# unixpickle/learn-nerf

Measured on AMD Instinct MI355X. Metric: ray-samples/s (NeRF train step: fwd + bwd + Adam, 4096 rays x 192 samples per GPU), higher is better.
Workload: dtype bf16; 1 GPU; vanilla NeRF coarse64+fine128 train step (BASELINE.json configs[1]); rays_per_gpu=4096, coarse_samples=64, fine_samples=128, global_batch_rays=4096, parallelism=dp1, precision=bf16 MFMA, fp32 accumulate/master weights

## Files before the change

learn-nerf_amd/csrc/fused_chain.h:

```cpp
#pragma once
#include <utility>

#include "common.h"
#include "fast_math.h"
#include "nerf_wgrad.h"

namespace lnrf {
using namespace nl;

typedef __bf16 bf16x8 __attribute__((ext_vector_type(8)));
typedef float f32x16 __attribute__((ext_vector_type(16)));
typedef float f32x4 __attribute__((ext_vector_type(4)));
typedef short s16x4 __attribute__((ext_vector_type(4)));


template <class F, int... I>
__device__ __forceinline__ void static_for_impl(F&& f, std::integer_sequence<int, I...>) {
  (f(std::integral_constant<int, I>{}), ...);
}
template <int N, class F>
__device__ __forceinline__ void static_for(F&& f) {
  static_for_impl(f, std::make_integer_sequence<int, N>{});
}

constexpr int kThreads = kWaves * 64;
constexpr int kStageBytes = kStageFrags * kFragBytes;
constexpr int kSlots = 3;
constexpr int kRingBytes = kSlots * kStageBytes;
constexpr int kBiasLdsOff = kRingBytes;
constexpr int kFragAhead = 4;

extern __shared__ __attribute__((aligned(16))) char smem[];

#ifdef LNRF_TIMELINE
struct Timeline {
  unsigned long long* buf = nullptr;
  int n = 0;
  bool on = false;
  __device__ __forceinline__ void stamp() {
    if (on) {
      const unsigned long long t = __builtin_amdgcn_s_memtime();
      if ((threadIdx.x & 63) == 0) buf[(threadIdx.x >> 6) * 1024 + n] = t;
      ++n;
    }
  }
};
#define LNRF_TL_STAMP(ring) (ring).tl.stamp()
#else
#define LNRF_TL_STAMP(ring) ((void)0)
#endif

__device__ __forceinline__ bf16x8 bits_to_frag(uint4 v) { return __builtin_bit_cast(bf16x8, v); }
__device__ __forceinline__ uint4 frag_to_bits(bf16x8 v) { return __builtin_bit_cast(uint4, v); }
__device__ __forceinline__ bf16x8 zero_frag() { return bits_to_frag(make_uint4(0, 0, 0, 0)); }

struct TileCtx {
  int lane, wave, c, h;
  int64_t tile, m;
  bool valid;
};
template <int NW>
__device__ __forceinline__ TileCtx tile_ctx(int64_t M) {
  const int tid = threadIdx.x;
  const int lane = tid & 63;
  const int wave = __builtin_amdgcn_readfirstlane(tid >> 6);
  const int c = lane & 31, h = lane >> 5;
  const int64_t tile = (int64_t)blockIdx.x * NW + wave;
  const int64_t m = tile * kTileCols + c;
  return {lane, wave, c, h, tile, m, m < M};
}

typedef __attribute__((address_space(1))) char gchar;
typedef unsigned u32x4 __attribute__((ext_vector_type(4)));
__device__ __forceinline__ gchar* uniform_global(const void* p) {
  uint64_t a = reinterpret_cast<uint64_t>(p);
  asm("" : "+s"(a));
  return (gchar*)a;
}


template <int NSTAGES, class SEQ, int NW = kWaves>
struct Ring {
  static constexpr int kPerWave = kStageFrags / NW;
  const char* stream;
  int wave, lane;
  uint4 r[2][kPerWave];
  bf16x8 fifo[kFragAhead];
#ifdef LNRF_TIMELINE
  Timeline tl;
#endif

  template <int T>
  __device__ __forceinline__ void load() {
#pragma unroll
    for (int q = 0; q < kPerWave; ++q) {
      const int f = wave + NW * q;
      const gchar* frag = uniform_global(stream + ((int64_t)T * kStageFrags + f) * kFragBytes);
      const u32x4 v = *reinterpret_cast<const __attribute__((address_space(1))) u32x4*>(frag + (unsigned)(lane * 16));
      r[T & 1][q] = make_uint4(v[0], v[1], v[2], v[3]);
    }
  }
  template <int T>
  __device__ __forceinline__ void write() {
#pragma unroll
    for (int q = 0; q < kPerWave; ++q) {
      const int f = wave + NW * q;
      *reinterpret_cast<uint4*>(&smem[(T % kSlots) * kStageBytes + f * kFragBytes + lane * 16]) = r[T & 1][q];
    }
  }
  template <int G>
  __device__ __forceinline__ bf16x8 read_lds() const {
    constexpr int off = ((G / kStageFrags) % kSlots) * kStageBytes + (G % kStageFrags) * kFragBytes;
    return bits_to_frag(*reinterpret_cast<const uint4*>(&smem[off + lane * 16]));
  }
  __device__ __forceinline__ void prologue() {
    load<0>();
    if constexpr (NSTAGES > 1) load<1>();
    write<0>();
    if constexpr (NSTAGES > 1) write<1>();
    if constexpr (NSTAGES > 2) load<2>();
    if constexpr (NSTAGES > 3) load<3>();
    __syncthreads();
    if constexpr (NSTAGES > 2) write<2>();
    if constexpr (NSTAGES > 4) load<4>();
    static_for<kFragAhead>([&](auto i) {
      constexpr int c = decltype(i)::value;
      if constexpr (c < SEQ::count) fifo[c] = read_lds<SEQ::at(c)>();
    });
  }
  template <int T>
  __device__ __forceinline__ void advance() {
#ifdef LNRF_TIMELINE
    tl.stamp();
#endif
    __syncthreads();
#ifdef LNRF_TIMELINE
    tl.stamp();
#endif
    if constexpr (T + 2 < NSTAGES) write<T + 2>();
    if constexpr (T + 4 < NSTAGES) load<T + 4>();
  }
  template <int C>
  __device__ __forceinline__ bf16x8 next() {
    constexpr int g = SEQ::at(C);
    if constexpr (g % kStageFrags == 0 && g > 0) advance<g / kStageFrags>();
    const bf16x8 a = fifo[C % kFragAhead];
    if constexpr (C + kFragAhead < SEQ::count) fifo[C % kFragAhead] = read_lds<SEQ::at(C + kFragAhead)>();
    return a;
  }
};

template <int COUNT>
struct LinSeq {
  static constexpr int count = COUNT;
  static constexpr int at(int c) { return c; }
};

template <int NT>
__device__ __forceinline__ void stage_bias(const char* bias_g, int n) {
  const float* src = reinterpret_cast<const float*>(bias_g);
  float* dst = reinterpret_cast<float*>(&smem[kBiasLdsOff]);
  for (int i = threadIdx.x; i < n; i += NT) dst[i] = src[i];
}
__device__ __forceinline__ f32x16 bias_acc(int bias_row0, int h) {
  f32x16 acc;
  const float* b = reinterpret_cast<const float*>(&smem[kBiasLdsOff]) + bias_row0 + 4 * h;
#pragma unroll
  for (int g = 0; g < 4; ++g) {
    const float4 v = *reinterpret_cast<const float4*>(b + 8 * g);
    acc[4 * g + 0] = v.x;
    acc[4 * g + 1] = v.y;
    acc[4 * g + 2] = v.z;
    acc[4 * g + 3] = v.w;
  }
  return acc;
}
__device__ __forceinline__ f32x16 zero_acc() {
  f32x16 acc;
#pragma unroll
  for (int q = 0; q < 16; ++q) acc[q] = 0.0f;
  return acc;
}

typedef __bf16 bf16x2 __attribute__((ext_vector_type(2)));
typedef float f32x2 __attribute__((ext_vector_type(2)));
typedef short s16x2 __attribute__((ext_vector_type(2)));
template <int S, bool RELU>
__device__ __forceinline__ bf16x8 acc_to_frag(const f32x16& acc) {
  u32x4 w;
#pragma unroll
  for (int p = 0; p < 4; ++p) {
    const f32x2 v = {acc[8 * S + 2 * p], acc[8 * S + 2 * p + 1]};
    bf16x2 b = __builtin_convertvector(v, bf16x2);
    if (RELU) {
      const s16x2 zero = {0, 0};
      b = __builtin_bit_cast(bf16x2, __builtin_elementwise_max(__builtin_bit_cast(s16x2, b), zero));
    }
    w[p] = __builtin_bit_cast(unsigned, b);
  }
  return __builtin_bit_cast(bf16x8, w);
}

__device__ __forceinline__ unsigned relu_bits(const bf16x8& f0, const bf16x8& f1) {
  const uint4 a = frag_to_bits(f0), b = frag_to_bits(f1);
  const unsigned w[8] = {a.x, a.y, a.z, a.w, b.x, b.y, b.z, b.w};
  unsigned bits = 0u;
#pragma unroll
  for (int i = 0; i < 8; ++i) {
    bits |= ((w[i] & 0xFFFFu) != 0u ? 1u : 0u) << (2 * i);
    bits |= ((w[i] >> 16) != 0u ? 1u : 0u) << (2 * i + 1);
  }
  return bits;
}
template <int S>
__device__ __forceinline__ bf16x8 masked_frag(const f32x16& acc, unsigned bits, int shift) {
  bf16x8 f;
#pragma unroll
  for (int j = 0; j < 8; ++j) f[j] = (__bf16)(((bits >> (shift + 8 * S + j)) & 1u) ? acc[8 * S + j] : 0.0f);
  return f;
}

__device__ __forceinline__ void store_tile_row(float* row, int h, const f32x16& acc) {
  float* zr = row + 4 * h;
#pragma unroll
  for (int g = 0; g < 4; ++g)
    *reinterpret_cast<float4*>(zr + 8 * g) = make_float4(acc[4 * g], acc[4 * g + 1], acc[4 * g + 2], acc[4 * g + 3]);
}
__device__ __forceinline__ void stream_store(gchar* p, uint4 v) {
  u32x4 t = {v.x, v.y, v.z, v.w};
  __builtin_nontemporal_store(t, reinterpret_cast<__attribute__((address_space(1))) u32x4*>(p));
}

__device__ __forceinline__ int64_t dump_off(int slot, int64_t tile, int64_t n_tiles, int n_slots) {
  if (n_slots > 0) return (tile * n_slots + slot) * kFragBytes;
  return ((int64_t)slot * n_tiles + tile) * kFragBytes;
}
struct DumpAddr {
  char* base;
  int64_t n_tiles;
  int64_t tile;
  int c, hh;
  int n_slots;
  __device__ __forceinline__ gchar* at(int slot) const {
    const int slot0 = n_slots > 0 ? (slot & ~3) : slot;
    gchar* group = uniform_global(base + dump_off(slot0, tile, n_tiles, n_slots));
    return group + (unsigned)((slot - slot0) * kFragBytes + dump_lane_off(slot, c, hh));
  }
  __device__ __forceinline__ void store(int slot, uint4 v) const { stream_store(at(slot), v); }
};
__device__ __forceinline__ uint4* mask_at(const char* buf, int slot, int64_t tile, int64_t n_tiles, int n_slots, int lane) {
  return reinterpret_cast<uint4*>(const_cast<char*>(buf) + dump_off(slot, tile, n_tiles, n_slots) + lane * 16);
}
__device__ __forceinline__ unsigned mask_word(const uint4& mk, int o) {
  return (o >> 1) == 0 ? mk.x : ((o >> 1) == 1 ? mk.y : ((o >> 1) == 2 ? mk.z : mk.w));
}
struct WgLayout {
  int x_slots, y_slots;
  int interleave = 0;
};

template <int C0, int NK, int NO, class RING, class Init, class GetB, class Epi>
__device__ __forceinline__ void chain_layer(RING& ring, Init init, GetB getb, Epi epi) {
  static_for<NO>([&](auto o_) {
    constexpr int o = decltype(o_)::value;
    f32x16 acc = init(o_);
    static_for<NK>([&](auto k_) {
      constexpr int ks = decltype(k_)::value;
      const bf16x8 a = ring.template next<C0 + o * NK + ks>();
      acc = __builtin_amdgcn_mfma_f32_32x32x16_bf16(a, getb(k_), acc, 0, 0, 0);
      __builtin_amdgcn_sched_barrier(0);
    });
    LNRF_TL_STAMP(ring);
    epi(o_, acc);
    LNRF_TL_STAMP(ring);
  });
}

constexpr int kSplitWaves = 4;
constexpr int kSplitThreads = kSplitWaves * 64;
template <int S, bool RELU>
__device__ __forceinline__ void acc_to_frag_split(const f32x16& acc, bf16x8& hi, bf16x8& lo) {
#pragma unroll
  for (int j = 0; j < 8; ++j) {
    float v = acc[8 * S + j];
    if (RELU) v = __builtin_amdgcn_fmed3f(v, 0.0f, __builtin_inff());
    const __bf16 hb = (__bf16)v;
    hi[j] = hb;
    lo[j] = (__bf16)(v - (float)hb);
  }
}
__device__ __forceinline__ void split_store(float v, bf16x8& hi, bf16x8& lo, int j) {
  const __bf16 hb = (__bf16)v;
  hi[j] = hb;
  lo[j] = (__bf16)(v - (float)hb);
}

__device__ __forceinline__ float param_or_zero(const float* params, int64_t idx) {
  return idx >= 0 ? params[idx] : 0.0f;
}
__device__ __forceinline__ __bf16 split_half(float w, bool lo_part) {
  const __bf16 hi = (__bf16)w;
  return lo_part ? (__bf16)(w - (float)hi) : hi;
}
template <int C0, int NK, int NO, class RING, class Init, class GetHi, class GetLo, class Epi>
__device__ __forceinline__ void chain_layer_split(RING& ring, Init init, GetHi bhi, GetLo blo, Epi epi) {
  static_for<NO>([&](auto o_) {
    constexpr int o = decltype(o_)::value;
    f32x16 acc = init(o_);
    static_for<NK>([&](auto k_) {
      constexpr int ks = decltype(k_)::value;
      constexpr int c = 2 * (C0 + o * NK + ks);
      const bf16x8 ahi = ring.template next<c>();
      const bf16x8 alo = ring.template next<c + 1>();
      acc = __builtin_amdgcn_mfma_f32_32x32x16_bf16(alo, bhi(k_), acc, 0, 0, 0);
      acc = __builtin_amdgcn_mfma_f32_32x32x16_bf16(ahi, blo(k_), acc, 0, 0, 0);
      acc = __builtin_amdgcn_mfma_f32_32x32x16_bf16(ahi, bhi(k_), acc, 0, 0, 0);
      __builtin_amdgcn_sched_barrier(0);
    });
    epi(o_, acc);
  });
}


__device__ __forceinline__ bf16x8 tr_frag(const char* frag_even, int lane, int parity, int q) {
  const int g = lane >> 4;
  const int i = lane & 15;
  const int frag = g & 1;
  const int hk = g >> 1;
  const int qp = i >> 2, p = i & 3;
  const int slot_par = parity ^ frag;
  const int c0 = 16 * q + 8 * hk;
  const int ca = c0 + qp, cb = c0 + 4 + qp;
  const char* base = frag_even + frag * kFragBytes;
  const int offa = 256 * (ca >> 3) + 128 * (((ca >> 2) & 1) ^ slot_par) + 64 * (p & 1) + 16 * (ca & 3) + 8 * (p >> 1);
  const int offb = 256 * (cb >> 3) + 128 * (((cb >> 2) & 1) ^ slot_par) + 64 * (p & 1) + 16 * (cb & 3) + 8 * (p >> 1);
  const s16x4 lo = __builtin_amdgcn_ds_read_tr16_b64_v4i16((__attribute__((address_space(3))) s16x4*)(base + offa));
  const s16x4 hi = __builtin_amdgcn_ds_read_tr16_b64_v4i16((__attribute__((address_space(3))) s16x4*)(base + offb));
  typedef short s16x8 __attribute__((ext_vector_type(8)));
  s16x8 v;
  v[0] = lo[0]; v[1] = lo[1]; v[2] = lo[2]; v[3] = lo[3];
  v[4] = hi[0]; v[5] = hi[1]; v[6] = hi[2]; v[7] = hi[3];
  return __builtin_bit_cast(bf16x8, v);
}

template <int NXF, int NYF, int SPI, bool PLAIN = false>
struct WgStage {
  static constexpr int kWgSpi = SPI;
  static constexpr int NF = NXF + NYF;
  static constexpr int PER_WAVE = (NF + kWaves - 1) / kWaves;
  static constexpr int STEP_BYTES = NF * kFragBytes;
  static constexpr int ITER_BYTES = kWgSpi * STEP_BYTES;
  const char* x_base;
  const char* y_base;
  int x_slot0, y_slot0, x_slots, y_slots;
  int64_t t0, n_tiles;
  int64_t iter_stride, t_end;
  int wave, lane;
  uint4 rr[kWgSpi][PER_WAVE];

  __device__ __forceinline__ void load(int64_t iter) {
    const int64_t tb = t0 + iter * iter_stride;
    const int64_t tbc = tb < t_end ? tb : t0;
    const int64_t xo = dump_off(x_slot0, tbc, n_tiles, x_slots), yo = dump_off(y_slot0, tbc, n_tiles, y_slots);
    const __amdgpu_buffer_rsrc_t rx = __builtin_amdgcn_make_buffer_rsrc(const_cast<char*>(x_base) + xo, 0, 0x7FFFFFFF, 0x00020000);
    const __amdgpu_buffer_rsrc_t ry = __builtin_amdgcn_make_buffer_rsrc(const_cast<char*>(y_base) + yo, 0, 0x7FFFFFFF, 0x00020000);
#pragma unroll
    for (int u = 0; u < kWgSpi; ++u) {
      const int64_t tl = tb + u;
      const bool ok = tl < t_end;
      const int64_t ta = ok ? tl : tbc;
      const unsigned keep = ok ? 0xFFFFFFFFu : 0u;
#pragma unroll
      for (int q = 0; q < PER_WAVE; ++q) {
        int f = wave + kWaves * q;
        if constexpr (NF % kWaves != 0) f = f < NF ? f : NF - 1;
        const bool isx = f < NXF;
        const int bo = (int)(isx ? dump_off(x_slot0 + f, ta, n_tiles, x_slots) - xo
                                 : dump_off(y_slot0 + f - NXF, ta, n_tiles, y_slots) - yo);
        const u32x4 v = __builtin_amdgcn_raw_buffer_load_b128(isx ? rx : ry, bo + lane * 16, 0, PLAIN ? 0 : 2);
        rr[u][q] = make_uint4(v[0] & keep, v[1] & keep, v[2] & keep, v[3] & keep);
      }
    }
  }
  template <int B>
  __device__ __forceinline__ void write() {
#pragma unroll
    for (int u = 0; u < kWgSpi; ++u) {
#pragma unroll
      for (int q = 0; q < PER_WAVE; ++q) {
        int f = wave + kWaves * q;
        if constexpr (NF % kWaves != 0) f = f < NF ? f : NF - 1;
        *reinterpret_cast<uint4*>(&smem[B * ITER_BYTES + u * STEP_BYTES + f * kFragBytes + lane * 16]) = rr[u][q];
      }
    }
  }
};

template <int NXF, int NYF, int WI, int WO, int SPI, bool PLAIN, class PB>
__device__ __forceinline__ void wgrad_body(const PB& pb, const char* __restrict__ save,
                                           const char* __restrict__ gdump, int64_t n_tiles,
                                           WgLayout lay, float* __restrict__ slabs) {
  constexpr int NI = NXF / 2, NO = NYF / 2;
  constexpr int TI = (NI + WI - 1) / WI, TO = (NO + WO - 1) / WO;
  constexpr bool FULL_I = TI * WI == NI, FULL_O = TO * WO == NO;
  using Stage = WgStage<NXF, NYF, SPI, PLAIN>;
  constexpr int kWgSpi = SPI;
  static_assert(WI * WO == kWaves, "wave grid");
  static_assert(NXF % 2 == 0 && NYF % 2 == 0, "fragment pairs");

  const int split = blockIdx.x - pb.first_block;

  const int tid = threadIdx.x;
  const int lane = tid & 63;
  const int wave = __builtin_amdgcn_readfirstlane(tid >> 6);
  const int wi = wave / WO, wo = wave % WO;

  const int64_t per = (n_tiles + pb.n_blocks - 1) / pb.n_blocks;
  int64_t t0 = (int64_t)split * per;
  const int64_t t1 = t0 + per < n_tiles ? t0 + per : n_tiles;
  const int64_t steps = t1 > t0 ? t1 - t0 : 0;
  int64_t iters = (steps + kWgSpi - 1) / kWgSpi;
  int64_t iter_stride = kWgSpi, t_end = t1;
  if (lay.interleave) {
    t0 = (int64_t)split * kWgSpi;
    iter_stride = (int64_t)pb.n_blocks * kWgSpi;
    t_end = n_tiles;
    iters = t0 < n_tiles ? (n_tiles - t0 + iter_stride - 1) / iter_stride : 0;
  }

  Stage stg;
  stg.x_base = save;
  stg.y_base = gdump;
  stg.x_slot0 = pb.x_slot0;
  stg.y_slot0 = pb.y_slot0;
  stg.x_slots = lay.x_slots;
  stg.y_slots = lay.y_slots;
  stg.t0 = t0;
  stg.n_tiles = n_tiles;
  stg.iter_stride = iter_stride;
  stg.t_end = t_end;
  stg.wave = wave;
  stg.lane = lane;

  f32x16 acc[TI][TO];
#pragma unroll
  for (int a = 0; a < TI; ++a)
#pragma unroll
    for (int b = 0; b < TO; ++b) acc[a][b] = zero_acc();
  float bsum[TO];
#pragma unroll
  for (int b = 0; b < TO; ++b) bsum[b] = 0.0f;
  const int ypar = pb.y_slot0 & 1, xpar = pb.x_slot0 & 1;

  auto compute = [&](auto buf_) {
    constexpr int bufi = decltype(buf_)::value;
#pragma unroll
    for (int u = 0; u < kWgSpi; ++u) {
      const char* buf = smem + bufi * Stage::ITER_BYTES + u * Stage::STEP_BYTES;
#pragma unroll
      for (int q = 0; q < 2; ++q) {
        bf16x8 bf[TO];
#pragma unroll
        for (int b = 0; b < TO; ++b) {
          const int ot = wo + WO * b;
          if (FULL_O || ot < NO) {
            bf[b] = tr_frag(buf + (NXF + 2 * ot) * kFragBytes, lane, ypar, q);
            if (wi == 0) {
#pragma unroll
              for (int j = 0; j < 8; ++j) bsum[b] += (float)bf[b][j];
            }
          }
        }
#pragma unroll
        for (int a = 0; a < TI; ++a) {
          const int it = wi + WI * a;
          if (FULL_I || it < NI) {
            const bf16x8 af = tr_frag(buf + 2 * it * kFragBytes, lane, xpar, q);
#pragma unroll
            for (int b = 0; b < TO; ++b) {
              const int ot = wo + WO * b;
              if (FULL_O || ot < NO)
                acc[a][b] = __builtin_amdgcn_mfma_f32_32x32x16_bf16(af, bf[b], acc[a][b], 0, 0, 0);
            }
          }
        }
      }
    }
  };
  std::integral_constant<int, 0> c0;
  std::integral_constant<int, 1> c1;
  if (iters > 0) {
    stg.load(0);
    stg.template write<0>();
    stg.load(1);
  }
  for (int64_t i = 0; i < iters; i += 2) {
    __syncthreads();
    stg.template write<1>();
    stg.load(i + 2);
    compute(c0);
    __syncthreads();
    stg.template write<0>();
    stg.load(i + 3);
    if (i + 1 < iters) compute(c1);
  }

  float* __restrict__ mine = slabs + ((int64_t)blockIdx.x * kWaves + wave) * kSlabWaveFloats;
#pragma unroll
  for (int a = 0; a < TI; ++a)
#pragma unroll
    for (int b = 0; b < TO; ++b) {
      float4* dst = reinterpret_cast<float4*>(mine + (a * TO + b) * kSlabTileFloats) + lane;
#pragma unroll
      for (int v = 0; v < 4; ++v)
        dst[64 * v] = make_float4(acc[a][b][4 * v], acc[a][b][4 * v + 1], acc[a][b][4 * v + 2], acc[a][b][4 * v + 3]);
    }
  if (wi == 0) {
#pragma unroll
    for (int b = 0; b < TO; ++b) mine[kSlabTileFloats * kSlabMaxTiles + b * 64 + lane] = bsum[b];
  }
}

constexpr int kSlabReduceWaves = 4;
template <int NXF, int NYF, int WI, int WO, class EPI, class PB>
__device__ __forceinline__ void wgrad_reduce_tile(const PB& pb, int w, int j, const float* __restrict__ slabs,
                                                  float* __restrict__ grads, float* lds) {
  if (j >= kWgradWaveTiles<NXF, NYF, WI, WO>) return;
  const int lane = threadIdx.x & 63, q = threadIdx.x >> 6;
  const WgradTile tile = wgrad_tile<NXF, NYF, WI, WO>(w, j);
  if (!tile.real) return;
  const int b = tile.b;
  const float* __restrict__ src = slabs + ((int64_t)pb.first_block * kWaves + w) * kSlabWaveFloats;
  const int64_t blk_stride = (int64_t)kWaves * kSlabWaveFloats;
  float acc[16];
#pragma unroll
  for (int r = 0; r < 16; ++r) acc[r] = 0.0f;
  const bool bias = tile.bias && pb.do_bias;
  float bsum = 0.0f;
  constexpr int U = 4;
  for (int s0 = q; s0 < pb.n_blocks; s0 += U * kSlabReduceWaves) {
    float4 t[U][4];
    float bb[U];
#pragma unroll
    for (int u = 0; u < U; ++u) {
      const int sb = s0 + u * kSlabReduceWaves;
      const int sblk = sb < pb.n_blocks ? sb : pb.n_blocks - 1;
      const float* base = src + (int64_t)sblk * blk_stride;
      const float4* tp = reinterpret_cast<const float4*>(base + j * kSlabTileFloats) + lane;
#pragma unroll
      for (int v = 0; v < 4; ++v) t[u][v] = tp[64 * v];
      bb[u] = bias ? base[kSlabTileFloats * kSlabMaxTiles + b * 64 + lane] : 0.0f;
    }
#pragma unroll
    for (int u = 0; u < U; ++u) {
      const bool ok = s0 + u * kSlabReduceWaves < pb.n_blocks;
#pragma unroll
      for (int v = 0; v < 4; ++v) {
        acc[4 * v] += ok ? t[u][v].x : 0.0f;
        acc[4 * v + 1] += ok ? t[u][v].y : 0.0f;
        acc[4 * v + 2] += ok ? t[u][v].z : 0.0f;
        acc[4 * v + 3] += ok ? t[u][v].w : 0.0f;
      }
      bsum += ok ? bb[u] : 0.0f;
    }
  }
  if (q > 0) {
#pragma unroll
    for (int r = 0; r < 16; ++r) lds[((q - 1) * 17 + r) * 64 + lane] = acc[r];
    lds[((q - 1) * 17 + 16) * 64 + lane] = bsum;
  }
  __syncthreads();
  if (q > 0) return;
#pragma unroll
  for (int p = 0; p < kSlabReduceWaves - 1; ++p) {
#pragma unroll
    for (int r = 0; r < 16; ++r) acc[r] += lds[(p * 17 + r) * 64 + lane];
    bsum += lds[(p * 17 + 16) * 64 + lane];
// ... 18 lines not shown
```

learn-nerf_amd/csrc/layout_host.cpp:

```cpp
#include <stdint.h>

#include "dense_plan.h"
#include "fast_math.h"
#include "nerf_wgrad.h"
#include "ngp_layout.h"

using namespace lnrf;

static WgradList wgrad_list_of(int which, int64_t n_tiles) {
  return which == 0 ? wgrad_list_split(n_tiles) : which == 1 ? wgrad_list_ls_finish(n_tiles)
       : which == 2 ? wgrad_list_ref_trunk(n_tiles) : which == 3 ? wgrad_list_ref_normal(n_tiles)
                                                                 : wgrad_list_ref_dir(n_tiles);
}
template <int NXF, int NYF, int WI, int WO>
static int64_t wgrad_count_owners(const WgradProblem& pb, int32_t* count, int64_t n) {
  int64_t outside = 0;
  int64_t i;
  auto hit = [&](bool owned) {
    if (!owned) return;
    if (i >= 0 && i < n) ++count[i];
    else ++outside;
  };
  for (int w = 0; w < kWaves; ++w)
    for (int j = 0; j < kWgradWaveTiles<NXF, NYF, WI, WO>; ++j) {
      const WgradTile tile = wgrad_tile<NXF, NYF, WI, WO>(w, j);
      if (!tile.real) continue;
      for (int lane = 0; lane < 64; ++lane) {
        const int colr = lane & 31, hh = lane >> 5;
        const WgradOwner<NerfWgradEpi, WgradProblem> own(pb, tile.ot, colr);
        if (tile.bias && pb.do_bias) hit(own.bias(hh, i));
        for (int qq = 0; qq < 16; ++qq) hit(own.weight(pb, tile.it, hh, qq, i));
      }
    }
  return outside;
}

template <int P>
static int64_t ngp_count_owners(const NgpWgradProblem& pb, int64_t dense_off, int32_t* count, int64_t n) {
  constexpr int NO = kNgpWgrad[P].nyf / 2, NT = ngp_wgrad_tiles(P);
  int64_t outside = 0;
  auto hit = [&](int part, int64_t i) {
    if (i >= 0 && i < n) ++count[part * n + i];
    else ++outside;
  };
  for (int w4 = 0; w4 < 4; ++w4)
    for (int lane = 0; lane < 64; ++lane) {
      const int colr = lane & 31, hh = lane >> 5;
      const int tile_id = w4 % NT, part = w4 / NT;
      const int it = tile_id / NO, ot = tile_id % NO;
      int out_idx = -1, out_dim = 1;
      int64_t w_off = 0, b_off = 0;
      NgpWgradEpi::cols(pb, ot, colr, out_idx, out_dim, w_off, b_off);
      w_off -= dense_off;
      b_off -= dense_off;
      if (it == 0 && hh == 0 && out_idx >= 0) hit(part, b_off + out_idx);
      for (int qq = 0; qq < 16; ++qq) {
        const int r = ngp_acc_row(qq, hh);
        const int f = 2 * it + (r >> 4);
        const int in_idx = NgpWgradEpi::row(pb, f, r & 15);
        if (out_idx >= 0 && in_idx >= 0) hit(part, w_off + (int64_t)in_idx * out_dim + out_idx);
      }
    }
  return outside;
}
static bool ngp_enc_dim_ok(int enc_dim) { return enc_dim >= 1 && enc_dim <= 32; }

extern "C" {
int lnrf_host_fwd_frags(void) { return kFwdFrags; }
int lnrf_host_bwd_frags(void) { return kBwdFrags; }
int lnrf_host_bias_floats(void) { return kBiasFloats; }
int lnrf_host_fwd_used(void) { return kFwdUsed; }
int lnrf_host_fwd_seq(int c) { return fwd_seq(c); }
int lnrf_host_fwd3_frags(void) { return kFwd3Frags; }
int lnrf_host_fwd3_used(void) { return kFwd3Used; }
int lnrf_host_fwd3_seq(int c) { return fwd3_seq(c); }
int lnrf_host_fwd3_base(int s) { return fwd3_base(s); }
int lnrf_host_bwd_seq(int c) { return bwd_seq(c); }
int lnrf_host_fwd_layer_info(int s, int what) {
  return what == 0 ? fwd_nk(s) : what == 1 ? fwd_no(s) : what == 2 ? fwd_base(s) : what == 3 ? fwd_bias_base(s)
                                                                                             : fwd_cons_base(s);
}
int lnrf_host_bwd_layer_info(int t, int what) {
  return what == 0 ? bwd_nk(t) : what == 1 ? bwd_no(t) : what == 2 ? bwd_base(t) : bwd_dense(t);
}
int lnrf_host_fwd_weight_index(int g, int lane, int j) { return fwd_stream_index(g, lane, j, false); }
int lnrf_host_bwd_weight_index(int g, int lane, int j) { return bwd_stream_index(g, lane, j, false); }
int lnrf_host_fwd_bias_index(int i) { return bias_block_index(i, false); }
int lnrf_host_nrm_frags(void) { return kNrmFrags; }
int lnrf_host_nrm_weight_index(int g, int lane, int j) { return nrm_stream_index(g, lane, j); }
int64_t lnrf_host_stream_indices(int stream, int ref, int32_t* out) {
  const int frags[8] = {kFwdFrags, kBwdFrags, kFwd3Frags, 0, kNrmFrags, kDirFwdFrags, kDirBwdFrags, 0};
  if (stream < 0 || stream > 7) return -1;
  if (stream == 3 || stream == 7) {
    const int n = stream == 3 ? kBiasFloats : kDirBiasFloats;
    for (int i = 0; out && i < n; ++i) out[i] = stream == 3 ? bias_block_index(i, ref != 0) : dir_bias_index(i);
    return n;
  }
  const int64_t n = (int64_t)frags[stream] * 512;
  for (int64_t e = 0; out && e < n; ++e) {
    const int g = (int)(e >> 9), lane = (int)((e >> 3) & 63), j = (int)(e & 7);
    out[e] = stream == 0 ? fwd_stream_index(g, lane, j, ref != 0) : stream == 1 ? bwd_stream_index(g, lane, j, ref != 0)
           : stream == 2 ? fwd3_stream_index(g, lane, j, ref != 0) : stream == 4 ? nrm_stream_index(g, lane, j)
           : stream == 5 ? dir_fwd_weight_index(g, lane, j) : dir_bwd_weight_index(g, lane, j);
  }
  return n;
}
int64_t lnrf_host_pack_offset(int what) {
  const int64_t v[17] = {kPackFwdOff, kPackBwdOff, kPackBiasOff, kPackBytes, kPack3BiasOff, kPack3Bytes,
                         kRefPackNrmOff, kRefPackDirFwdOff, kRefPackDirBwdOff, kRefPackDirBiasOff, kRefPackBytes,
                         kRef3FwdOff, kRef3BiasOff, kRef3NrmOff, kRef3DirOff, kRef3DirBiasOff, kRef3Bytes};
  return what >= 0 && what < 17 ? v[what] : -1;
}
int lnrf_host_xemb_feat(int ks, int h, int j) { return xemb_feat(ks, h, j); }
int lnrf_host_save_slot(int what, int arg) {
  return what == 0 ? kSaveXin : what == 1 ? kSaveH + 16 * arg : what == 2 ? kSaveZ : what == 3 ? kSaveDin
       : what == 4 ? kSaveH10 : what == 5 ? kSaveMask : kSaveSlots;
}
int lnrf_host_grad_slot(int what, int arg) {
  return what == 0 ? kGradDy11 : what == 1 ? kGradDy10m : what == 2 ? grad_dy_slot(arg) : kGradSlots;
}
int lnrf_host_dir_slot(int what) {
  const int v[7] = {kDirSaveXin, kDirSaveH, kDirSaveMask, kDirSaveSlots, kDirGradDy10, kDirGradDy9, kDirGradSlots};
  return what >= 0 && what < 7 ? v[what] : -1;
}
int lnrf_host_demb_feat(int ks, int h, int j) { return demb_feat(ks, h, j); }
int lnrf_host_hidden_feat(int ks, int h, int j) { return hidden_feat(ks, h, j); }
int lnrf_host_dump_info(int what) { return what == 0 ? kFragBytes : what == 1 ? kTileCols : kWaves; }
int lnrf_host_mask_bit(int ks, int j) { return 16 * (ks >> 1) + 8 * (ks & 1) + j; }
int lnrf_host_dump_lane_off(int slot, int c, int hh) { return dump_lane_off(slot, c, hh); }
void lnrf_host_sincos_pe(float r, float* s, float* c) { lnrf::sincos_pe(r, s, c); }

int lnrf_host_wgrad_const(int what) {
  const int v[8] = {kWgradMaxBlocks, kSlabMaxTiles, kSlabMaxTO, kParamCount, kDirW9, kDirB9, kDirW10, kDirB10};
  return v[what];
}
int lnrf_host_wgrad_list(int which, int64_t n_tiles, int32_t* out) {
  const WgradList list = wgrad_list_of(which, n_tiles);
  for (int i = 0; i < list.args.n_problems; ++i) {
    const WgradProblem& pb = list.args.p[i];
    int32_t* o = out + 6 * i;
    o[0] = pb.first_block; o[1] = pb.n_blocks; o[4] = pb.do_bias; o[5] = 0;
    switch (pb.shape) {
#define X(name, id, NXF, NYF, WI, WO, SPI) case name: o[2] = WgShape<name>::TI * WgShape<name>::TO; o[3] = WgShape<name>::TO; break;
      LNRF_WGRAD_SHAPES(X, X)
#undef X
      default: return -1;
    }
    switch (pb.shape) {
#define X(name) case name:
      LNRF_WGRAD_LS_SHAPES(X, X) o[5] = 1; break;
#undef X
      default: break;
    }
  }
  return list.args.n_problems;
}
int64_t lnrf_host_ngp_stream_indices(int stream, int enc_dim, int32_t* out) {
  if (stream < 0 || stream > 2 || !ngp_enc_dim_ok(enc_dim)) return -1;
  const NgpOffsets off = ngp_offsets(enc_dim, 0);
  const int ne = ngp_ne(enc_dim);
  const int64_t n = stream == 2 ? kNgpBiasFloats : (int64_t)kNgpStreamFrags * 512;
  for (int64_t e = 0; out && e < n; ++e) {
    const int g = (int)(e >> 9), lane = (int)((e >> 3) & 63), j = (int)(e & 7);
    out[e] = (int32_t)(stream == 0 ? ngp_fwd_stream_index(g, lane, j, off, enc_dim, ne)
                     : stream == 1 ? ngp_bwd_stream_index(g, lane, j, off, enc_dim, ne) : ngp_bias_index((int)e, off));
  }
  return n;
}
int64_t lnrf_host_ngp_pack_offset(int what) {
  const int64_t v[7] = {kNgpPackBiasOff, kNgpPackBytes, kNgpSplitBiasOff, kNgpSplitBytes, kNgpStreamFrags,
                        kNgpSplitMaxFrags / 2, kNgpMaxParts};
  return what >= 0 && what < 7 ? v[what] : -1;
}
int64_t lnrf_host_ngp_wgrad_owners(int enc_dim, int32_t* count, int64_t n) {
  if (!ngp_enc_dim_ok(enc_dim)) return -1;
  const int64_t dense_off = 1001;
  const NgpWgradArgs a = ngp_wgrad_args(ngp_offsets(enc_dim, dense_off), enc_dim);
  return ngp_count_owners<0>(a.p[0], dense_off, count, n) + ngp_count_owners<1>(a.p[1], dense_off, count, n) +
         ngp_count_owners<2>(a.p[2], dense_off, count, n) + ngp_count_owners<3>(a.p[3], dense_off, count, n) +
         ngp_count_owners<4>(a.p[4], dense_off, count, n);
}
int lnrf_host_ngp_parts_plan(int enc_dim, int32_t* out) {
  if (!ngp_enc_dim_ok(enc_dim)) return -1;
  const NgpPartsPlan pl = ngp_parts_plan(ngp_offsets(enc_dim, 1001), 1001);
  for (int i = 0; i < kNgpLayers; ++i) {
    int32_t* o = out + 4 * i;
    o[0] = kNgpWgrad[i].layer; o[1] = pl.lo[i]; o[2] = pl.hi[i]; o[3] = pl.parts[i];
  }
  return ngp_dense_params(enc_dim);
}
void lnrf_host_gemm_plan(int64_t sa_i, int64_t sa_r, int64_t sb_r, int64_t sb_j, int64_t I, int32_t J, int64_t R,
                         uint32_t a_low, uint32_t b_low, int32_t bf16, int32_t mode, int32_t splits, int64_t* out) {
  const GemmPlan p = gemm_plan(sa_i, sa_r, sb_r, sb_j, I, J, R, a_low, b_low, bf16 != 0, mode, splits);
  const int64_t v[15] = {p.launch, p.big, p.bf16, p.a_fast_r, p.b_fast_r, p.b_aligned, p.kc, p.nsplit, p.lda, p.ldb,
                         p.r_per_split, p.gx, p.gy, p.gz, p.splits};
  for (int i = 0; i < 15; ++i) out[i] = v[i];
}
void lnrf_host_gemm_tile(int64_t I, int32_t J, uint32_t block0, int64_t count, int64_t* out) {
  for (int64_t e = 0; e < count; ++e) {
    const GemmTile t = gemm_big_tile(block0 + (uint32_t)e, (I + BI - 1) / BI, (J + BJ - 1) / BJ);
    out[2 * e] = t.it;
    out[2 * e + 1] = t.jt;
  }
}
int64_t lnrf_host_dense_bwd_weight_scratch_bytes(int64_t m, int32_t k, int32_t n) { return dense_wgrad_scratch_bytes(m, k, n); }
int64_t lnrf_host_gemm_det_scratch_bytes(int64_t I, int32_t J, int64_t R) { return gemm_det_scratch_bytes(I, J, R); }
int64_t lnrf_host_wgrad_owners(int which, int64_t n_tiles, int32_t* count, int64_t n) {
  const WgradList list = wgrad_list_of(which, n_tiles);
  int64_t outside = 0;
  for (int i = 0; i < list.args.n_problems; ++i) {
    const WgradProblem& pb = list.args.p[i];
    switch (pb.shape) {
#define X(name, id, NXF, NYF, WI, WO, SPI) case name: outside += wgrad_count_owners<NXF, NYF, WI, WO>(pb, count, n); break;
      LNRF_WGRAD_SHAPES(X, X)
#undef X
    }
  }
  return outside;
}
}
```

learn-nerf_amd/csrc/nerf_mlp.hip:

```cpp
#include "nerf_chain.h"

namespace lnrf {

constexpr int kFusedLds = kRingBytes + round_up(kBiasFloats * 4, 1024);
#ifdef LNRF_TIMELINE
__device__ unsigned long long* g_timeline_buf = nullptr;
#endif

struct FwdSeq {
  static constexpr int count = kFwdUsed;
  static constexpr int at(int c) { return fwd_seq(c); }
};

constexpr int kFwdStages = kFwdFrags / kStageFrags;

template <bool SAVE, bool FROM_RAYS, bool HMASKS = true>
__global__ __launch_bounds__(kThreads) void nerf_fwd_kernel(
    const char* __restrict__ packed, const float* __restrict__ xin_g, const float* __restrict__ din_g,
    const float* __restrict__ rays, int64_t ray_stride, const float* __restrict__ ts, int T, int64_t M,
    int64_t n_tiles, float* __restrict__ density, float* __restrict__ rgb, char* __restrict__ save) {
  const auto [lane, wave, c, h, tile, m, valid] = tile_ctx<kWaves>(M);

  stage_bias<kThreads>(packed + kPackBiasOff, kBiasFloats);
  float px[3] = {0, 0, 0}, pd[3] = {0, 0, 0};
  if (valid) {
    if (FROM_RAYS) {
      const int64_t n = m / T;
      const float t = ts[m];
      const float* r = rays + n * ray_stride;
#pragma unroll
      for (int a = 0; a < 3; ++a) {
        pd[a] = r[3 + a];
        px[a] = r[a] + pd[a] * t;
      }
    } else {
#pragma unroll
      for (int a = 0; a < 3; ++a) {
        px[a] = xin_g[m * 3 + a];
        pd[a] = din_g[m * 3 + a];
      }
    }
  }
  __syncthreads();

  Ring<kFwdStages, FwdSeq> ring;
  ring.stream = packed + kPackFwdOff;
  ring.wave = wave;
  ring.lane = lane;
#ifdef LNRF_TIMELINE
  ring.tl.buf = g_timeline_buf + (SAVE ? 0 : 8 * 1024);
  ring.tl.n = 0;
  ring.tl.on = g_timeline_buf != nullptr && blockIdx.x == gridDim.x / 2;
  ring.tl.stamp();
#endif
  ring.prologue();
  LNRF_TL_STAMP(ring);

  bf16x8 xe[4], de[2];
  x_encode(px, h, [&](auto ks_, int j, float v) { xe[decltype(ks_)::value][j] = (__bf16)v; });
  static_for<2>([&](auto ks_) {
    constexpr int ks = decltype(ks_)::value;
#pragma unroll
    for (int pp = 0; pp < 4; ++pp) {
      const int p = 4 * ks + pp;
      float s = 0.0f, co = 0.0f;
      if (p < 6) {
        const int pg = 6 * h + p;
        const int cd = pg >> 2, f = pg & 3;
        const float v = cd == 0 ? pd[0] : (cd == 1 ? pd[1] : pd[2]);
        sincos_pe(v * (float)(1 << f), &s, &co);
      }
      de[ks][2 * pp] = (__bf16)s;
      de[ks][2 * pp + 1] = (__bf16)co;
    }
  });

  DumpAddr dump{save, n_tiles, tile, c, h, kSaveTileSlots};
  auto save_frag = [&](int slot, const bf16x8& f) {
    if (SAVE) dump.store(slot, frag_to_bits(f));
  };
  if (SAVE) {
    static_for<4>([&](auto i) { save_frag(kSaveXin + decltype(i)::value, xe[decltype(i)::value]); });
    static_for<2>([&](auto i) { save_frag(kSaveDin + decltype(i)::value, de[decltype(i)::value]); });
  }

  bf16x8 a0[16], a1[16];
  unsigned mask_bits[4] = {0u, 0u, 0u, 0u};

  auto hidden = [&](auto s_, bf16x8(&in)[16], bf16x8(&out)[16], auto relu_, int save_slot) {
    constexpr int S = decltype(s_)::value;
    constexpr bool RELU = decltype(relu_)::value;
    trunk_layer<S, true>(ring, h, xe, in, [&](auto o_, const f32x16& acc) {
      constexpr int o = decltype(o_)::value;
      out[2 * o] = acc_to_frag<0, RELU>(acc);
      out[2 * o + 1] = acc_to_frag<1, RELU>(acc);
      save_frag(save_slot + 2 * o, out[2 * o]);
      save_frag(save_slot + 2 * o + 1, out[2 * o + 1]);
      if constexpr (SAVE && RELU && HMASKS)
        mask_bits[o >> 1] |= relu_bits(out[2 * o], out[2 * o + 1]) << (16 * (o & 1));
    });
    if constexpr (SAVE && RELU && HMASKS) {
      *mask_at(save, kSaveMask + S, tile, n_tiles, kSaveTileSlots, lane) =
          make_uint4(mask_bits[0], mask_bits[1], mask_bits[2], mask_bits[3]);
      mask_bits[0] = mask_bits[1] = mask_bits[2] = mask_bits[3] = 0u;
    }
  };
  std::true_type relu;
  std::false_type lin;
  hidden(std::integral_constant<int, 0>{}, a1, a0, relu, kSaveH + 0 * 16);
  hidden(std::integral_constant<int, 1>{}, a0, a1, relu, kSaveH + 1 * 16);
  hidden(std::integral_constant<int, 2>{}, a1, a0, relu, kSaveH + 2 * 16);
  hidden(std::integral_constant<int, 3>{}, a0, a1, relu, kSaveH + 3 * 16);
  hidden(std::integral_constant<int, 4>{}, a1, a0, relu, kSaveH + 4 * 16);
  hidden(std::integral_constant<int, 5>{}, a0, a1, relu, kSaveH + 5 * 16);
  hidden(std::integral_constant<int, 6>{}, a1, a0, relu, kSaveH + 6 * 16);
  hidden(std::integral_constant<int, 7>{}, a0, a1, relu, kSaveH + 7 * 16);
  hidden(std::integral_constant<int, 8>{}, a1, a0, lin, kSaveZ);

  chain_layer<fwd_cons_base(9), fwd_nk(9), fwd_no(9)>(
      ring, [&](auto o_) { return bias_acc(fwd_bias_base(9) + 32 * decltype(o_)::value, h); },
      [&](auto k_) -> bf16x8 {
        constexpr int ks = decltype(k_)::value;
        if constexpr (ks < 16) return a0[ks];
        else return de[ks - 16];
      },
      [&](auto o_, const f32x16& acc) {
        constexpr int o = decltype(o_)::value;
        if constexpr (o < 4) {
          a1[2 * o] = acc_to_frag<0, true>(acc);
          a1[2 * o + 1] = acc_to_frag<1, true>(acc);
          save_frag(kSaveH10 + 2 * o, a1[2 * o]);
          save_frag(kSaveH10 + 2 * o + 1, a1[2 * o + 1]);
          if constexpr (SAVE) mask_bits[o >> 1] |= relu_bits(a1[2 * o], a1[2 * o + 1]) << (16 * (o & 1));
        } else {
          if constexpr (SAVE)
            *mask_at(save, kSaveMask + 8, tile, n_tiles, kSaveTileSlots, lane) = make_uint4(mask_bits[0], mask_bits[1], 0u, 0u);
          if (h == 0 && valid) {
            const float x = acc[0];
            density[m] = fmaxf(x, 0.0f) + log1pf(expf(-fabsf(x)));
          }
        }
      });
  chain_layer<fwd_cons_base(10), fwd_nk(10), fwd_no(10)>(
      ring, [&](auto) { return bias_acc(fwd_bias_base(10), h); },
      [&](auto k_) -> bf16x8 { return a1[decltype(k_)::value]; },
      [&](auto, const f32x16& acc) {
        if (h == 0 && valid) {
          rgb[m * 3 + 0] = tanhf(acc[0]);
          rgb[m * 3 + 1] = tanhf(acc[1]);
          rgb[m * 3 + 2] = tanhf(acc[2]);
        }
      });
}

constexpr int kFwd3Stages = kFwd3Frags / kStageFrags;
struct Fwd3Seq {
  static constexpr int count = kFwd3Used;
  static constexpr int at(int c) { return fwd3_seq(c); }
};

template <bool FROM_RAYS>
__global__ __launch_bounds__(kSplitThreads) void nerf_fwd_split_kernel(
    const char* __restrict__ packed, const float* __restrict__ xin_g, const float* __restrict__ din_g,
    const float* __restrict__ rays, int64_t ray_stride, const float* __restrict__ ts, int T, int64_t M,
    float* __restrict__ density, float* __restrict__ rgb) {
  const auto [lane, wave, c, h, tile, m, valid] = tile_ctx<kSplitWaves>(M);

  stage_bias<kSplitThreads>(packed + kPack3BiasOff, kBiasFloats);
  float px[3] = {0, 0, 0}, pd[3] = {0, 0, 0};
  if (valid) {
    if (FROM_RAYS) {
      const int64_t n = m / T;
      const float t = ts[m];
      const float* r = rays + n * ray_stride;
#pragma unroll
      for (int a = 0; a < 3; ++a) {
        pd[a] = r[3 + a];
        px[a] = r[a] + pd[a] * t;
      }
    } else {
#pragma unroll
      for (int a = 0; a < 3; ++a) {
        px[a] = xin_g[m * 3 + a];
        pd[a] = din_g[m * 3 + a];
      }
    }
  }
  __syncthreads();

  Ring<kFwd3Stages, Fwd3Seq, kSplitWaves> ring;
  ring.stream = packed;
  ring.wave = wave;
  ring.lane = lane;
  ring.prologue();

  bf16x8 xe_hi[4], xe_lo[4], de_hi[2], de_lo[2];
  x_encode(px, h, [&](auto ks_, int j, float v) { split_store(v, xe_hi[decltype(ks_)::value], xe_lo[decltype(ks_)::value], j); });
  static_for<2>([&](auto ks_) {
    constexpr int ks = decltype(ks_)::value;
#pragma unroll
    for (int pp = 0; pp < 4; ++pp) {
      const int p = 4 * ks + pp;
      float s = 0.0f, co = 0.0f;
      if (p < 6) {
        const int pg = 6 * h + p;
        const int cd = pg >> 2, f = pg & 3;
        const float v = cd == 0 ? pd[0] : (cd == 1 ? pd[1] : pd[2]);
        sincos_pe(v * (float)(1 << f), &s, &co);
      }
      split_store(s, de_hi[ks], de_lo[ks], 2 * pp);
      split_store(co, de_hi[ks], de_lo[ks], 2 * pp + 1);
    }
  });

  bf16x8 a0h[16], a0l[16], a1h[16], a1l[16];

  auto hidden = [&](auto s_, bf16x8(&inh)[16], bf16x8(&inl)[16], bf16x8(&outh)[16], bf16x8(&outl)[16], auto relu_) {
    constexpr bool RELU = decltype(relu_)::value;
    trunk_layer_split<decltype(s_)::value>(ring, h, xe_hi, xe_lo, inh, inl, [&](auto o_, const f32x16& acc) {
      constexpr int o = decltype(o_)::value;
      acc_to_frag_split<0, RELU>(acc, outh[2 * o], outl[2 * o]);
      acc_to_frag_split<1, RELU>(acc, outh[2 * o + 1], outl[2 * o + 1]);
    });
  };
  std::true_type relu;
  std::false_type lin;
  hidden(std::integral_constant<int, 0>{}, a1h, a1l, a0h, a0l, relu);
  hidden(std::integral_constant<int, 1>{}, a0h, a0l, a1h, a1l, relu);
  hidden(std::integral_constant<int, 2>{}, a1h, a1l, a0h, a0l, relu);
  hidden(std::integral_constant<int, 3>{}, a0h, a0l, a1h, a1l, relu);
  hidden(std::integral_constant<int, 4>{}, a1h, a1l, a0h, a0l, relu);
  hidden(std::integral_constant<int, 5>{}, a0h, a0l, a1h, a1l, relu);
  hidden(std::integral_constant<int, 6>{}, a1h, a1l, a0h, a0l, relu);
  hidden(std::integral_constant<int, 7>{}, a0h, a0l, a1h, a1l, relu);
  hidden(std::integral_constant<int, 8>{}, a1h, a1l, a0h, a0l, lin);

  chain_layer_split<fwd_cons_base(9), fwd_nk(9), fwd_no(9)>(
      ring, [&](auto o_) { return bias_acc(fwd_bias_base(9) + 32 * decltype(o_)::value, h); },
      [&](auto k_) -> bf16x8 {
        constexpr int ks = decltype(k_)::value;
        if constexpr (ks < 16) return a0h[ks];
        else return de_hi[ks - 16];
      },
      [&](auto k_) -> bf16x8 {
        constexpr int ks = decltype(k_)::value;
        if constexpr (ks < 16) return a0l[ks];
        else return de_lo[ks - 16];
      },
      [&](auto o_, const f32x16& acc) {
        constexpr int o = decltype(o_)::value;
        if constexpr (o < 4) {
          acc_to_frag_split<0, true>(acc, a1h[2 * o], a1l[2 * o]);
          acc_to_frag_split<1, true>(acc, a1h[2 * o + 1], a1l[2 * o + 1]);
        } else {
          if (h == 0 && valid) {
            const float x = acc[0];
            density[m] = fmaxf(x, 0.0f) + log1pf(expf(-fabsf(x)));
          }
        }
      });
  chain_layer_split<fwd_cons_base(10), fwd_nk(10), fwd_no(10)>(
      ring, [&](auto) { return bias_acc(fwd_bias_base(10), h); },
      [&](auto k_) -> bf16x8 { return a1h[decltype(k_)::value]; },
      [&](auto k_) -> bf16x8 { return a1l[decltype(k_)::value]; },
      [&](auto, const f32x16& acc) {
        if (h == 0 && valid) {
          rgb[m * 3 + 0] = tanhf(acc[0]);
          rgb[m * 3 + 1] = tanhf(acc[1]);
          rgb[m * 3 + 2] = tanhf(acc[2]);
        }
      });
}

__global__ __launch_bounds__(kThreads) void nerf_bwd_chain_kernel(
    const char* __restrict__ packed, const char* __restrict__ save, const float* __restrict__ density,
    const float* __restrict__ rgb, const float* __restrict__ g_density, const float* __restrict__ g_rgb,
    int64_t M, int64_t n_tiles, char* __restrict__ gdump) {
  const auto [lane, wave, c, h, tile, m, valid] = tile_ctx<kWaves>(M);

  Ring<kBwdStages, BwdSeq> ring;
  ring.stream = packed + kPackBwdOff;
  ring.wave = wave;
  ring.lane = lane;
#ifdef LNRF_TIMELINE
  ring.tl.buf = g_timeline_buf + 16 * 1024;
  ring.tl.n = 0;
  ring.tl.on = g_timeline_buf != nullptr && blockIdx.x == gridDim.x / 2;
  ring.tl.stamp();
#endif
  const DumpAddr gd{gdump, n_tiles, tile, c, h, kGradTileSlots};
  bwd_chain_tile(ring, gd, save, n_tiles, density, rgb, g_density, g_rgb, M, tile, lane);
}

template <bool PLAIN>
__global__ __launch_bounds__(kThreads) void nerf_wgrad_kernel(WgradArgs args, const char* __restrict__ save,
                                                              const char* __restrict__ gdump, int64_t n_tiles,
                                                              WgLayout lay, float* __restrict__ slabs) {
  WgradProblem pb = args.p[0];
#pragma unroll
  for (int i = 1; i < kMaxProblems; ++i)
    if (i < args.n_problems && (int)blockIdx.x >= args.p[i].first_block) pb = args.p[i];
  switch (pb.shape) {
#define X(name, id, NXF, NYF, WI, WO, SPI) \
  case name: wgrad_body<NXF, NYF, WI, WO, SPI, PLAIN>(pb, save, gdump, n_tiles, lay, slabs); break;
    LNRF_WGRAD_SHAPES(X, default: X)
#undef X
  }
}

__global__ __launch_bounds__(64 * kSlabReduceWaves) void nerf_wgrad_reduce_kernel(WgradArgs args,
                                                                                 const float* __restrict__ slabs,
                                                                                 float* __restrict__ grads) {
  __shared__ float lds[(kSlabReduceWaves - 1) * 17 * 64];
  const int prob = blockIdx.x / (kWaves * kSlabMaxTiles), w = blockIdx.x / kSlabMaxTiles % kWaves, j = blockIdx.x % kSlabMaxTiles;
  const WgradProblem pb = args.p[prob];
  switch (pb.shape) {
#define X(name, id, NXF, NYF, WI, WO, SPI) \
  case name: wgrad_reduce_tile<NXF, NYF, WI, WO, NerfWgradEpi>(pb, w, j, slabs, grads, lds); break;
    LNRF_WGRAD_SHAPES(X, default: X)
#undef X
  }
}

__global__ void nerf_pack_kernel(const float* __restrict__ params, char* __restrict__ packed) {
  constexpr int64_t units_f = (int64_t)kFwdFrags * 64, units_b = (int64_t)kBwdFrags * 64;
  constexpr int64_t total = units_f + units_b + kBiasFloats;
  for (int64_t u = (int64_t)blockIdx.x * blockDim.x + threadIdx.x; u < total; u += (int64_t)gridDim.x * blockDim.x) {
    if (u < units_f + units_b) {
      const bool fwd = u < units_f;
      const int64_t uu = fwd ? u : u - units_f;
      const int g = (int)(uu >> 6), lane = (int)(uu & 63);
      bf16x8 out;
#pragma unroll
      for (int j = 0; j < 8; ++j)
        out[j] = (__bf16)param_or_zero(params, fwd ? fwd_stream_index(g, lane, j, false) : bwd_stream_index(g, lane, j, false));
      *reinterpret_cast<bf16x8*>(packed + (fwd ? kPackFwdOff : kPackBwdOff) + uu * 16) = out;
    } else {
      const int i = (int)(u - units_f - units_b);
      reinterpret_cast<float*>(packed + kPackBiasOff)[i] = param_or_zero(params, bias_block_index(i, false));
    }
  }
}

__global__ void nerf_pack_split_kernel(const float* __restrict__ params, char* __restrict__ packed) {
  const int64_t total_w = (int64_t)kFwd3Frags * 512;
  const int64_t total = total_w + kBiasFloats;
  for (int64_t e = (int64_t)blockIdx.x * blockDim.x + threadIdx.x; e < total;
       e += (int64_t)gridDim.x * blockDim.x) {
// ... 196 lines not shown
```

Before: 187.2 million ray-samples/s.

## Alternate wave-group phases in the forward weight ring with open/close barriers

Adds a phase table to the forward-pass weight ring so that, in the layers whose K equals one stage, the barrier is split into an open barrier (before the stage's fragments are consumed) and a close barrier (after the output tile's MFMAs), and the two halves of the waves are offset by extra one-sided barriers at layer boundaries. The write of a future stage and the global load of a later stage are moved to different barrier points. The aim is to stagger the two wave groups so LDS reads and MFMA work overlap better and barrier stalls are hidden. It only applies to the SAVE forward variant and adds more barriers per layer, which risks extra synchronization cost. A host-side event walker is also added for inspection.

```diff
diff --git a/learn-nerf_amd/csrc/fused_chain.h b/learn-nerf_amd/csrc/fused_chain.h
--- a/learn-nerf_amd/csrc/fused_chain.h
+++ b/learn-nerf_amd/csrc/fused_chain.h
@@ -4,6 +4,7 @@
 #include "common.h"
 #include "fast_math.h"
 #include "nerf_wgrad.h"
+#include "ring_phase.h"
 
 namespace lnrf {
 using namespace nl;
@@ -25,10 +26,8 @@
 
 constexpr int kThreads = kWaves * 64;
 constexpr int kStageBytes = kStageFrags * kFragBytes;
-constexpr int kSlots = 3;
 constexpr int kRingBytes = kSlots * kStageBytes;
 constexpr int kBiasLdsOff = kRingBytes;
-constexpr int kFragAhead = 4;
 
 extern __shared__ __attribute__((aligned(16))) char smem[];
 
@@ -37,18 +36,21 @@
   unsigned long long* buf = nullptr;
   int n = 0;
   bool on = false;
-  __device__ __forceinline__ void stamp() {
+  __device__ __forceinline__ void stamp(int tag = 0) {
     if (on) {
-      const unsigned long long t = __builtin_amdgcn_s_memtime();
+      const unsigned long long t = (__builtin_amdgcn_s_memtime() & 0x00FFFFFFFFFFFFFFull) | ((unsigned long long)tag << 56);
       if ((threadIdx.x & 63) == 0) buf[(threadIdx.x >> 6) * 1024 + n] = t;
       ++n;
     }
   }
 };
 #define LNRF_TL_STAMP(ring) (ring).tl.stamp()
+#define LNRF_TL_TAG(ring, tag) (ring).tl.stamp(tag)
 #else
 #define LNRF_TL_STAMP(ring) ((void)0)
+#define LNRF_TL_TAG(ring, tag) ((void)0)
 #endif
+constexpr int kTlArrive = 0x40, kTlRelease = 0x80, kTlMfma = 0x20, kTlEpi = 0x21;
 
 __device__ __forceinline__ bf16x8 bits_to_frag(uint4 v) { return __builtin_bit_cast(bf16x8, v); }
 __device__ __forceinline__ uint4 frag_to_bits(bf16x8 v) { return __builtin_bit_cast(uint4, v); }
@@ -79,7 +81,7 @@
 }
 
 
-template <int NSTAGES, class SEQ, int NW = kWaves>
+template <int NSTAGES, class SEQ, int NW = kWaves, class PH = NoPhase>
 struct Ring {
   static constexpr int kPerWave = kStageFrags / NW;
   const char* stream;
@@ -131,19 +133,57 @@
   template <int T>
   __device__ __forceinline__ void advance() {
 #ifdef LNRF_TIMELINE
-    tl.stamp();
+    tl.stamp(kTlArrive | kPhStage);
 #endif
     __syncthreads();
 #ifdef LNRF_TIMELINE
-    tl.stamp();
+    tl.stamp(kTlRelease | kPhStage);
 #endif
     if constexpr (T + 2 < NSTAGES) write<T + 2>();
     if constexpr (T + 4 < NSTAGES) load<T + 4>();
   }
+  __device__ __forceinline__ void phase_barrier(int kind) {
+    LNRF_TL_TAG(*this, kTlArrive | kind);
+    __builtin_amdgcn_sched_barrier(0);
+    __syncthreads();
+    __builtin_amdgcn_sched_barrier(0);
+    LNRF_TL_TAG(*this, kTlRelease | kind);
+  }
+  template <int C, int T>
+  __device__ __forceinline__ void phase_pre() {
+    constexpr int kind = PH::pre(C);
+    static_assert(!(kind & (kPhStage | kPhOpen)) == !(SEQ::at(C) % kStageFrags == 0 && SEQ::at(C) > 0),
+                  "a stage starts exactly where the table has a stage or an open barrier");
+    if constexpr ((kind & kPhExtraHi) != 0) {
+      if (wave >= NW / 2) phase_barrier(kPhExtraHi);
+    }
+    if constexpr ((kind & kPhExtraLo) != 0) {
+      if (wave < NW / 2) phase_barrier(kPhExtraLo);
+    }
+    if constexpr ((kind & kPhOpen) != 0) {
+      phase_barrier(kPhOpen);
+      if constexpr (T + kWriteAhead < NSTAGES) write<T + kWriteAhead>();
+    } else if constexpr ((kind & kPhStage) != 0) {
+      phase_barrier(kPhStage);
+      if constexpr (T + kWriteAhead < NSTAGES) write<T + kWriteAhead>();
+      if constexpr (T + kLoadAhead < NSTAGES) load<T + kLoadAhead>();
+    }
+  }
+  template <int C>
+  __device__ __forceinline__ void after() {
+    if constexpr (PH::on) {
+      if constexpr ((PH::post(C) & kPhClose) != 0) {
+        constexpr int T = SEQ::at(C) / kStageFrags;
+        phase_barrier(kPhClose);
+        if constexpr (T + kLoadAhead < NSTAGES) load<T + kLoadAhead>();
+      }
+    }
+  }
   template <int C>
   __device__ __forceinline__ bf16x8 next() {
     constexpr int g = SEQ::at(C);
-    if constexpr (g % kStageFrags == 0 && g > 0) advance<g / kStageFrags>();
+    if constexpr (PH::on) phase_pre<C, g / kStageFrags>();
+    else if constexpr (g % kStageFrags == 0 && g > 0) advance<g / kStageFrags>();
     const bf16x8 a = fifo[C % kFragAhead];
     if constexpr (C + kFragAhead < SEQ::count) fifo[C % kFragAhead] = read_lds<SEQ::at(C + kFragAhead)>();
     return a;
@@ -270,9 +310,10 @@
       acc = __builtin_amdgcn_mfma_f32_32x32x16_bf16(a, getb(k_), acc, 0, 0, 0);
       __builtin_amdgcn_sched_barrier(0);
     });
-    LNRF_TL_STAMP(ring);
+    LNRF_TL_TAG(ring, kTlMfma);
+    ring.template after<C0 + o * NK + NK - 1>();
     epi(o_, acc);
-    LNRF_TL_STAMP(ring);
+    LNRF_TL_TAG(ring, kTlEpi);
   });
 }
 
diff --git a/learn-nerf_amd/csrc/layout_host.cpp b/learn-nerf_amd/csrc/layout_host.cpp
--- a/learn-nerf_amd/csrc/layout_host.cpp
+++ b/learn-nerf_amd/csrc/layout_host.cpp
@@ -4,6 +4,7 @@
 #include "fast_math.h"
 #include "nerf_wgrad.h"
 #include "ngp_layout.h"
+#include "ring_phase.h"
 
 using namespace lnrf;
 
@@ -65,7 +66,52 @@
 }
 static bool ngp_enc_dim_ok(int enc_dim) { return enc_dim >= 1 && enc_dim <= 32; }
 
+template <class Emit>
+static void fwd_ring_walk(int group, Emit emit) {
+  constexpr int n_stages = kFwdFrags / kStageFrags;
+  emit(4, 0), emit(4, 1), emit(1, 0), emit(1, 1), emit(4, 2), emit(4, 3);
+  emit(0, -1);
+  emit(1, 2), emit(4, 4);
+  for (int c = 0; c < kFragAhead && c < kFwdUsed; ++c) emit(2, fwd_seq(c));
+  for (int c = 0; c < kFwdUsed; ++c) {
+    const int pre = FwdPhase::pre(c), post = FwdPhase::post(c), t = fwd_seq(c) / kStageFrags;
+    if ((pre & kPhExtraHi) && group == 1) emit(0, kPhExtraHi);
+    if ((pre & kPhExtraLo) && group == 0) emit(0, kPhExtraLo);
+    if (pre & (kPhOpen | kPhStage)) {
+      emit(0, pre & (kPhOpen | kPhStage));
+      if (t + kWriteAhead < n_stages) emit(1, t + kWriteAhead);
+      if ((pre & kPhStage) && t + kLoadAhead < n_stages) emit(4, t + kLoadAhead);
+    }
+    if (c + kFragAhead < kFwdUsed) emit(2, fwd_seq(c + kFragAhead));
+    emit(3, c);
+    if (post & kPhClose) {
+      emit(0, kPhClose);
+      if (t + kLoadAhead < n_stages) emit(4, t + kLoadAhead);
+    }
+  }
+}
+
 extern "C" {
+int lnrf_host_ring_const(int what) {
+  const int v[10] = {kSlots, kFragAhead, kWriteAhead, kLoadAhead, kStageFrags, kPhStage, kPhOpen, kPhClose, kPhExtraHi, kPhExtraLo};
+  return what >= 0 && what < 10 ? v[what] : -1;
+}
+int lnrf_host_fwd_phase_pre(int c) { return c >= 0 && c < kFwdUsed ? fwd_phase_pre(c) : -1; }
+int lnrf_host_fwd_phase_post(int c) { return c >= 0 && c < kFwdUsed ? fwd_phase_post(c) : -1; }
+int lnrf_host_fwd_cons_layer(int c) { return c >= 0 && c < kFwdUsed ? fwd_cons_layer(c) : -1; }
+int lnrf_host_fwd_alternates(int s) { return fwd_alternates(s) ? 1 : 0; }
+int lnrf_host_fwd_ring_events(int group, int32_t* out, int cap) {
+  int n = 0;
+  fwd_ring_walk(group, [&](int ev, int arg) { ++n; });
+  if (out == nullptr || cap < n) return n;
+  int i = 0;
+  fwd_ring_walk(group, [&](int ev, int arg) {
+    out[2 * i] = ev;
+    out[2 * i + 1] = arg;
+    ++i;
+  });
+  return n;
+}
 int lnrf_host_fwd_frags(void) { return kFwdFrags; }
 int lnrf_host_bwd_frags(void) { return kBwdFrags; }
 int lnrf_host_bias_floats(void) { return kBiasFloats; }
diff --git a/learn-nerf_amd/csrc/nerf_mlp.hip b/learn-nerf_amd/csrc/nerf_mlp.hip
--- a/learn-nerf_amd/csrc/nerf_mlp.hip
+++ b/learn-nerf_amd/csrc/nerf_mlp.hip
@@ -43,7 +43,11 @@
   }
   __syncthreads();
 
+#if defined(LNRF_TIMELINE) && defined(LNRF_TIMELINE_IN_PHASE)
   Ring<kFwdStages, FwdSeq> ring;
+#else
+  Ring<kFwdStages, FwdSeq, kWaves, std::conditional_t<SAVE, FwdPhase, NoPhase>> ring;
+#endif
   ring.stream = packed + kPackFwdOff;
   ring.wave = wave;
   ring.lane = lane;
diff --git a/learn-nerf_amd/csrc/ring_phase.h b/learn-nerf_amd/csrc/ring_phase.h
--- /dev/null
+++ b/learn-nerf_amd/csrc/ring_phase.h
@@ -0,0 +1,60 @@
+#pragma once
+#include "nerf_layout.h"
+
+namespace lnrf {
+namespace nl {
+
+constexpr int kSlots = 3;
+constexpr int kFragAhead = 4;
+constexpr int kWriteAhead = 2;
+constexpr int kLoadAhead = 4;
+
+constexpr int kPhNone = 0;
+constexpr int kPhStage = 1;
+constexpr int kPhOpen = 2;
+constexpr int kPhClose = 4;
+constexpr int kPhExtraHi = 8;
+constexpr int kPhExtraLo = 16;
+
+struct NoPhase {
+  static constexpr bool on = false;
+};
+
+NL_HD constexpr bool fwd_alternates(int s) {
+  return s >= 0 && s < kFwdLayers && fwd_nk(s) == kStageFrags && fwd_no(s) > 1 && fwd_base(s) % kStageFrags == 0;
+}
+NL_HD constexpr int fwd_cons_layer(int c) {
+  int s = 0;
+  for (int i = 1; i < kFwdLayers; ++i)
+    if (c >= fwd_cons_base(i)) s = i;
+  return s;
+}
+NL_HD constexpr int fwd_phase_pre(int c) {
+  const int s = fwd_cons_layer(c), loc = c - fwd_cons_base(s);
+  if (fwd_alternates(s)) {
+    if (loc % fwd_nk(s) != 0) return kPhNone;
+    return kPhOpen | (loc == 0 && !fwd_alternates(s - 1) ? kPhExtraHi : 0);
+  }
+  const int g = fwd_seq(c);
+  if (g == 0 || g % kStageFrags != 0) return kPhNone;
+  return kPhStage | (loc == 0 && fwd_alternates(s - 1) ? kPhExtraLo : 0);
+}
+NL_HD constexpr int fwd_phase_post(int c) {
+  const int s = fwd_cons_layer(c), loc = c - fwd_cons_base(s);
+  return fwd_alternates(s) && loc % fwd_nk(s) == fwd_nk(s) - 1 ? kPhClose : kPhNone;
+}
+struct FwdPhase {
+  static constexpr bool on = true;
+  static constexpr int pre(int c) { return fwd_phase_pre(c); }
+  static constexpr int post(int c) { return fwd_phase_post(c); }
+};
+static_assert(!fwd_alternates(0) && !fwd_alternates(kFwdLayers - 1), "the stream starts and ends with both groups in phase");
+static_assert(fwd_alternates(1) && fwd_alternates(4) && !fwd_alternates(5) && fwd_alternates(6) && fwd_alternates(8) &&
+                  !fwd_alternates(9),
+              "Dense_1..4 and Dense_6..8 alternate");
+static_assert((fwd_phase_pre(fwd_cons_base(5)) & kPhExtraLo) && (fwd_phase_pre(fwd_cons_base(9)) & kPhExtraLo) &&
+                  (fwd_phase_pre(fwd_cons_base(1)) & kPhExtraHi) && (fwd_phase_pre(fwd_cons_base(6)) & kPhExtraHi),
+              "every offset that is opened is closed");
+
+}
+}
```

After: 186.8 million ray-samples/s. Within noise of the previous version (-0.2%).
